# ekimb/rust-mdbg

Hardware: AMD Instinct MI355X
Metric: Gbases/s ingested to k-min-mer graph (higher is better)
Workload: dtype u64

## Files before the change

### include/mdbg_hip.h

```cpp
#ifndef MDBG_HIP_H
#define MDBG_HIP_H

#include <stddef.h>
#include <stdint.h>

#ifdef __cplusplus
extern "C" {
#endif

#define MDBG_ABI_VERSION 3

enum {
    MDBG_OK = 0,
    MDBG_E_PARAM = -1,
    MDBG_E_ALPHABET = -2,
    MDBG_E_CAPACITY = -3,
    MDBG_E_DEVICE = -4,
    MDBG_E_NOMEM = -5,
    MDBG_E_STATE = -6,
    MDBG_E_IO = -7
};

#define MDBG_MAX_L 255u
#define MDBG_MAX_MINABUND 65535u
// ... 183 lines not shown
    const uint64_t* step_offsets;
    const uint32_t* first_window; const uint32_t* step_windows; const uint32_t* unitig; const uint32_t* first_entry; const uint8_t* strand;
    const uint64_t* support_windows; const uint64_t* support_steps;
} mdbg_read_path_list;
int mdbg_graph_read_paths(mdbg_ctx* ctx, uint64_t first_read, uint64_t max_reads, mdbg_read_path_list* out);
int mdbg_graph_read_paths_device(mdbg_ctx* ctx, uint64_t first_read, uint64_t max_reads, mdbg_read_path_list* out);
int mdbg_read_paths_ms(mdbg_ctx* ctx, double* ms);

int mdbg_set_partition(mdbg_ctx* ctx, uint32_t world, uint32_t rank);
typedef struct mdbg_sketch_store {
    uint64_t n_minimizers, n_reads;
    const uint64_t* d_hashes;
    const uint32_t* d_positions;
    const uint64_t* d_read_offsets;
} mdbg_sketch_store;
int mdbg_sketch_view(mdbg_ctx* ctx, mdbg_sketch_store* out);
int mdbg_ingest_sketch(mdbg_ctx* ctx, const uint64_t* d_hashes, const uint32_t* d_positions, const uint64_t* d_read_offsets,
                       uint64_t n_reads, uint64_t first_read_ordinal);
int mdbg_store_reserve(mdbg_ctx* ctx, uint64_t n_minimizers_total, uint64_t n_reads_total);
int mdbg_sketch_reserve(mdbg_ctx* ctx, uint64_t n_minimizers, uint64_t** d_hashes, uint32_t** d_positions, uint64_t* region);
int mdbg_sketch_commit(mdbg_ctx* ctx, uint64_t region, uint64_t n_minimizers, const uint64_t* d_read_offsets, uint64_t n_reads,
                       uint64_t first_read_ordinal, uint64_t owned_windows);
int mdbg_owner_counts(mdbg_ctx* ctx, uint32_t world, uint64_t* counts);
int mdbg_owner_lists(mdbg_ctx* ctx, uint32_t world, uint64_t* counts, const uint32_t** d_lists);
int mdbg_sketch_commit_listed(mdbg_ctx* ctx, uint64_t region, uint64_t n_minimizers, const uint64_t* d_read_offsets, uint64_t n_reads,
                              uint64_t first_read_ordinal, const uint32_t* d_list, uint64_t n_list);
typedef struct mdbg_batch_info {
    uint64_t store_offset, n_minimizers, first_slot, n_reads, first_read_ordinal;
    const uint64_t* d_hashes;
    const uint32_t* d_positions;
    const uint64_t* d_read_offsets;
} mdbg_batch_info;
int mdbg_last_batch(mdbg_ctx* ctx, mdbg_batch_info* out);
int mdbg_finalize_begin(mdbg_ctx* ctx, uint64_t** d_bm_first, uint64_t** d_bm_solid, uint64_t* n_words);
int mdbg_finalize_end(mdbg_ctx* ctx, mdbg_nodes* out, const uint64_t** d_row, uint64_t* n_nodes_global);

int mdbg_sync(mdbg_ctx* ctx);
int mdbg_copy_to_host(mdbg_ctx* ctx, void* dst, const void* d_src, uint64_t nbytes);
int mdbg_copy_to_device(mdbg_ctx* ctx, void* d_dst, const void* src, uint64_t nbytes);

typedef struct mdbg_synth_params {
    uint64_t seed;
    uint64_t genome_len;
    uint64_t n_reads;
    uint32_t mean_len, sd_len, min_len, max_len;
    uint32_t err_ppm;
    uint32_t reserved;
} mdbg_synth_params;
int mdbg_synth_reads_device(mdbg_ctx* ctx, const mdbg_synth_params* sp, uint64_t first_read,
                            const uint8_t** d_bases, const uint64_t** d_offsets, uint64_t* n_bases);

int mdbg_dbg_segments_ms(mdbg_ctx* ctx, uint32_t world, uint32_t skip, const uint64_t* counts, const uint32_t* d_lists, double* out);

#ifdef __cplusplus
}
#endif
#endif
```

### rust_mdbg_amd/api.py

```python
import ctypes as C
import os

import numpy as np

_HERE = os.path.dirname(os.path.abspath(__file__))
_LIB = None

MDBG_OK, MDBG_E_PARAM, MDBG_E_ALPHABET, MDBG_E_CAPACITY, MDBG_E_DEVICE, MDBG_E_NOMEM, MDBG_E_STATE, MDBG_E_IO = 0, -1, -2, -3, -4, -5, -6, -7
FLAG_FORCE_GENERIC = 1
FLAG_KEEP_READS = 2


class MdbgError(RuntimeError):
    def __init__(self, code, msg):
        super().__init__("mdbg error %d: %s" % (code, msg))
        self.code = code


class Params(C.Structure):
    _fields_ = [("k", C.c_uint32), ("l", C.c_uint32), ("density", C.c_double), ("min_abundance", C.c_uint32),
                ("reads_already_hpc", C.c_uint32), ("device", C.c_int32), ("flags", C.c_uint32),
                ("table_capacity_hint", C.c_uint64), ("scheme", C.c_uint32), ("syncmer_s", C.c_uint32), ("reserved", C.c_uint64 * 3)]


# ... 89 lines not shown
                ("unitig", C.POINTER(C.c_uint64))]


class NodeSeqs(C.Structure):
    _fields_ = [("first_row", C.c_uint64), ("n_rows", C.c_uint64), ("n_bases", C.c_uint64), ("bases", C.POINTER(C.c_uint8)), ("offsets", C.POINTER(C.c_uint64))]


class SimplifyStep(C.Structure):
    _fields_ = [("kind", C.c_uint32), ("max_nodes", C.c_uint32), ("max_bases", C.c_uint64)]


class SimplifyStats(C.Structure):
    _fields_ = [("n_steps", C.c_uint32), ("n_compactions", C.c_uint32), ("unitigs_removed", C.POINTER(C.c_uint64)), ("nodes_removed", C.POINTER(C.c_uint64)),
                ("total_unitigs_removed", C.c_uint64), ("total_nodes_removed", C.c_uint64), ("n_rounds_total", C.c_uint32), ("n_syncs", C.c_uint32)]


MDBG_SIMPLIFY_TIPS, MDBG_SIMPLIFY_BUBBLES = 1, 2
MDBG_SIMPLIFY_COMPONENTS = 4
_T, _B = (MDBG_SIMPLIFY_TIPS, 10, 50000), (MDBG_SIMPLIFY_BUBBLES, 0, 100000)
MAGIC_SIMPLIFY_STEPS = [_T, _T, _B, _B, _T, _B, _B, _B, _T, _B, _T, (MDBG_SIMPLIFY_BUBBLES, 0, 1000000), (MDBG_SIMPLIFY_TIPS, 10, 150000),
                        (MDBG_SIMPLIFY_BUBBLES, 0, 1000000)]


def simplify_steps(steps):
    steps = [tuple(int(x) for x in s) for s in steps]
    if not steps:
        return None, 0
    return (SimplifyStep * len(steps))(*[SimplifyStep(k, mn, mb) for k, mn, mb in steps]), len(steps)


def unitig_name(i, circular):
    return "utg%07d%s" % (i + 1, "c" if circular else "l")


class PackedBatch(C.Structure):
    _fields_ = [("words", C.c_void_p), ("offsets", C.c_void_p), ("n_reads", C.c_uint64), ("exc_pos", C.c_void_p),
                ("exc_val", C.c_void_p), ("n_exc", C.c_uint64)]


class SynthParams(C.Structure):
    _fields_ = [("seed", C.c_uint64), ("genome_len", C.c_uint64), ("n_reads", C.c_uint64), ("mean_len", C.c_uint32),
                ("sd_len", C.c_uint32), ("min_len", C.c_uint32), ("max_len", C.c_uint32), ("err_ppm", C.c_uint32),
                ("reserved", C.c_uint32)]


EXPORTS = ["mdbg_abi_version", "mdbg_build_flags", "mdbg_create", "mdbg_destroy", "mdbg_finalize_device", "mdbg_finalize_gfa", "mdbg_nodes_digest", "mdbg_set_timing", "mdbg_ingest_batch", "mdbg_ingest_batch_device", "mdbg_sketch_only",
           "mdbg_finalize", "mdbg_reset", "mdbg_get_stats", "mdbg_strerror", "mdbg_last_error", "mdbg_sketch_device",
           "mdbg_insert_resident", "mdbg_route_pack", "mdbg_insert_records", "mdbg_sync", "mdbg_synth_reads_device", "mdbg_copy_to_host", "mdbg_copy_to_device",
           "mdbg_routed_export", "mdbg_resolve_first", "mdbg_resolve_meta", "mdbg_routed_keys", "mdbg_arena_reserve",
           "mdbg_set_partition", "mdbg_sketch_view", "mdbg_ingest_sketch", "mdbg_finalize_begin", "mdbg_finalize_end",
           "mdbg_store_reserve", "mdbg_sketch_reserve", "mdbg_sketch_commit", "mdbg_last_batch", "mdbg_owner_counts", "mdbg_graph_edges", "mdbg_graph_edges_device", "mdbg_graph_unitigs", "mdbg_graph_unitigs_device",
           "mdbg_graph_simplify", "mdbg_graph_simplify_device", "mdbg_graph_components", "mdbg_graph_components_device", "mdbg_graph_contigs", "mdbg_graph_contigs_device", "mdbg_kept_reads", "mdbg_contigs_ms", "mdbg_graph_node_seqs", "mdbg_graph_node_seqs_device", "mdbg_node_seqs_ms", "mdbg_graph_read_paths", "mdbg_graph_read_paths_device", "mdbg_read_paths_ms",
           "mdbg_ingest_batch_packed", "mdbg_ingest_batch_packed_device", "mdbg_sketch_packed_device", "mdbg_pack_device", "mdbg_query_batch", "mdbg_owner_lists", "mdbg_sketch_commit_listed", "mdbg_mark", "mdbg_rewind", "mdbg_set_lmer_filter",
           "mdbg_release_cached_memory", "mdbg_host_alloc", "mdbg_host_free", "mdbg_host_is_pinned", "mdbg_dbg_segments_ms"]


def lib_path():
    return os.path.join(_HERE, "libmdbg_hip.so")


def load_library():
    global _LIB
    if _LIB is not None:
        return _LIB
    p = lib_path()
    if not os.path.exists(p):
        raise ImportError("libmdbg_hip.so not built (%s); run `make -C rust_mdbg_amd/csrc`" % p)
    import sys
    if "torch" not in sys.modules and not os.environ.get("MDBG_NO_TORCH_PRELOAD"):
        import importlib.util
        if importlib.util.find_spec("torch") is not None:
            import torch
    L = C.CDLL(p)
    vp, u64, u32 = C.c_void_p, C.c_uint64, C.c_uint32
    L.mdbg_abi_version.restype = u32
    L.mdbg_build_flags.restype = u32
    L.mdbg_release_cached_memory.restype = u64
    L.mdbg_host_alloc.restype = vp
    L.mdbg_host_alloc.argtypes = [C.c_size_t]
    L.mdbg_host_free.restype = None
    L.mdbg_host_free.argtypes = [vp]
    L.mdbg_host_is_pinned.argtypes = [vp]
    L.mdbg_create.restype = vp
    L.mdbg_create.argtypes = [C.POINTER(Params), C.POINTER(C.c_int)]
    L.mdbg_destroy.restype = None
    L.mdbg_destroy.argtypes = [vp]
    L.mdbg_ingest_batch.argtypes = [vp, vp, vp, u64, u64]
    L.mdbg_ingest_batch_device.argtypes = [vp, vp, vp, u64, u64, u64]
    L.mdbg_sketch_device.argtypes = [vp, vp, vp, u64, u64, u64]
    L.mdbg_insert_resident.argtypes = [vp]
    L.mdbg_ingest_batch_packed.argtypes = [vp, C.POINTER(PackedBatch), u64]
    L.mdbg_ingest_batch_packed_device.argtypes = [vp, C.POINTER(PackedBatch), u64, u64]
    L.mdbg_sketch_packed_device.argtypes = [vp, C.POINTER(PackedBatch), u64, u64]
    L.mdbg_pack_device.argtypes = [vp, vp, u64, vp, vp, vp, u64, C.POINTER(u64)]
    L.mdbg_query_batch.argtypes = [vp, vp, vp, u64, C.POINTER(C.POINTER(u32)), C.POINTER(C.POINTER(u64)), C.POINTER(u64)]
    L.mdbg_query_batch.restype = C.c_int
    L.mdbg_sketch_only.argtypes = [vp, vp, vp, u64, C.POINTER(C.POINTER(u64)), C.POINTER(C.POINTER(u64)), C.POINTER(C.POINTER(u64)), C.POINTER(u64)]
    L.mdbg_finalize.argtypes = [vp, C.POINTER(Nodes)]
    L.mdbg_finalize_device.argtypes = [vp, C.POINTER(Nodes)]
    L.mdbg_finalize_gfa.argtypes = [vp, C.POINTER(Nodes)]
    L.mdbg_set_timing.argtypes = [vp, u32]
    L.mdbg_nodes_digest.argtypes = [vp, C.POINTER(Nodes), C.POINTER(C.c_uint64), C.POINTER(C.c_uint64)]
    L.mdbg_reset.argtypes = [vp, u32]
    L.mdbg_get_stats.argtypes = [vp, C.POINTER(Stats)]
    L.mdbg_strerror.restype = C.c_char_p
    L.mdbg_strerror.argtypes = [C.c_int]
    L.mdbg_last_error.restype = C.c_char_p
# ... 452 lines not shown
```

### rust_mdbg_amd/csrc/import_api.inc

```
int mdbg_set_partition(mdbg_ctx* c, uint32_t world, uint32_t rank) {
    if (!c) return MDBG_E_PARAM;
    MDBG_LOCK(c);
    if (world < 1 || world > 4096 || rank >= world) return fail(c, MDBG_E_PARAM, "bad partition");
    if (c->n_distinct || c->batches_inserted) return fail(c, MDBG_E_STATE, "set the partition before inserting");
    c->own_world = world; c->own_rank = rank;
    return MDBG_OK;
}

int mdbg_sketch_view(mdbg_ctx* c, mdbg_sketch_store* out) {
    if (!c || !out) return MDBG_E_PARAM;
    MDBG_LOCK(c);
    (void)hipSetDevice(c->dev);
    HIPCHK(c, hipStreamSynchronize(c->stream));
    out->n_minimizers = c->M; out->n_reads = c->n_slots;
    out->d_hashes = c->mh.as<u64>(); out->d_positions = c->mpos.as<u32>(); out->d_read_offsets = c->roff.as<u64>();
    return MDBG_OK;
}

int mdbg_ingest_sketch(mdbg_ctx* c, const uint64_t* d_hashes, const uint32_t* d_positions, const uint64_t* d_read_offsets, uint64_t n_reads,
                       uint64_t first_read_ordinal) {
    if (!c) return MDBG_E_PARAM;
    MDBG_LOCK(c);
    (void)hipSetDevice(c->dev);
    if (c->poisoned) return fail(c, MDBG_E_STATE, "context is in an error state");
// ... 159 lines not shown
}

static int batch_info_impl(mdbg_ctx* c, mdbg_batch_info* out, size_t which, bool sync = true) {
    if (!c || !out) return MDBG_E_PARAM;
    if (c->batches.empty() || (which != ~(size_t)0 && which >= c->batches.size())) return fail(c, MDBG_E_STATE, "no batch has been sketched or imported");
    MDBG_LOCK(c);
    (void)hipSetDevice(c->dev);
    if (sync) HIPCHK(c, hipStreamSynchronize(c->stream));
    const Batch& b = which == ~(size_t)0 ? c->batches.back() : c->batches[which];
    out->store_offset = b.m0; out->n_minimizers = b.m1 - b.m0; out->first_slot = b.slot0; out->n_reads = b.n_reads; out->first_read_ordinal = b.first_ordinal;
    out->d_hashes = c->mh.as<u64>() + b.m0; out->d_positions = c->mpos.as<u32>() + b.m0; out->d_read_offsets = c->roff.as<u64>() + b.slot0;
    return MDBG_OK;
}
int mdbg_last_batch(mdbg_ctx* c, mdbg_batch_info* out) { return batch_info_impl(c, out, ~(size_t)0); }

int mdbg_dbg_segments_ms(mdbg_ctx* c, uint32_t world, uint32_t skip, const uint64_t* counts, const uint32_t* d_lists, double* out) {
    if (!c || !counts || !d_lists || !out || world < 1 || world > OWNL_MAX_WORLD) return MDBG_E_PARAM;
    MDBG_LOCK(c);
    (void)hipSetDevice(c->dev);
    if (c->batches.empty()) return fail(c, MDBG_E_STATE, "no batch");
    const Batch& b = c->batches.back();
    hipStream_t s = c->stream;
    SegBuckets B{}; B.n = world; B.skip = skip;
    u64 total = 0;
    for (u32 r = 0; r < world; ++r) { B.start[r] = total; B.base[r] = b.m0; B.lim[r] = b.m1 - b.m0; total += counts[r]; }
    B.start[world] = total;
    out[0] = out[1] = 0; out[2] = (double)total; out[3] = 0;
    if (!total) return MDBG_OK;
    DevBuf tmp, misc, pay, scratch;
    HIPCHK(c, tmp.ensure((total / 1024 + 2) * 8, 0, s)); HIPCHK(c, misc.ensure((size_t)(OWNL_MAX_WORLD + 4) * 8, 0, s));
    HIPCHK(c, pay.ensure((b.m1 - b.m0) * 8 + 8, 0, s)); HIPCHK(c, scratch.ensure((b.m1 - b.m0) * 8 + 8, 0, s));
    hipEvent_t e0, e1; HIPCHK(c, hipEventCreate(&e0)); HIPCHK(c, hipEventCreate(&e1));
    u64 picks[OWNL_MAX_WORLD + 1] = {0};
    float best[2] = {1e30f, 1e30f};
    for (int rep = 0; rep < 3; ++rep)
        for (int side = 0; side < 2; ++side) {
            if (side) for (u32 r = 0; r < world; ++r) B.base[r] = 0;
            else for (u32 r = 0; r < world; ++r) B.base[r] = b.m0;
            HIPCHK(c, hipMemsetAsync(misc.p, 0, 8, s));
            HIPCHK(c, hipEventRecord(e0, s));
            launch_seg_prefix(d_lists, total, c->P.k, B, tmp.as<u64>(), misc.as<u64>(), misc.as<u64>() + 1, s);
            HIPCHK(c, hipMemcpyAsync(picks, misc.as<u64>() + 1, (size_t)(world + 1) * 8, hipMemcpyDeviceToHost, s));
            if (!side) HIPCHK(c, hipStreamSynchronize(s));
            launch_seg_copy(d_lists, total, c->P.k, B, tmp.as<u64>(), side ? scratch.as<u64>() : c->mh.as<u64>(), pay.as<u64>(), b.m1 - b.m0, side != 0, s);
            HIPCHK(c, hipEventRecord(e1, s));
            HIPCHK(c, hipStreamSynchronize(s));
            float ms = 0; HIPCHK(c, hipEventElapsedTime(&ms, e0, e1));
            if (ms < best[side]) best[side] = ms;
        }
    (void)hipEventDestroy(e0); (void)hipEventDestroy(e1);
    out[0] = best[0]; out[1] = best[1]; out[3] = (double)picks[world];
    return MDBG_OK;
}
```

### rust_mdbg_amd/csrc/owner.hip

```cpp
#include "mdbg_dev.h"
__global__ void owner_thresholds_kernel(double bound, u32 k, u32 world, u64* __restrict__ thr) {
    const u32 r = threadIdx.x + 1;
    if (threadIdx.x == 0) thr[0] = 0;
    thr += OWNER_THR_AT;
    if (r >= world) return;
    const double x = -expm1(log1p(-(double)r / (double)world) / (double)k);
    double v = x * bound;
    thr[r - 1] = v >= 18446744073709549568.0 ? ~0ull : (u64)v;
}
void launch_owner_thresholds(double bound, u32 k, u32 world, u64* thr, hipStream_t s) {
    if (world > 1) hipLaunchKernelGGL(owner_thresholds_kernel, dim3(1), dim3(64), 0, s, bound, k, world, thr);
}

__global__ __launch_bounds__(256) void count_owned_windows_kernel(const u64* __restrict__ mh, const u32* __restrict__ mread, const u64* __restrict__ roff, u64 i0, u64 i1,
                                                                  u32 k, u32 world, const u64* thr, u32 rank, u64* __restrict__ out) {
    constexpr int WPT = 4;
    const u64 b0 = i0 + (u64)blockIdx.x * (256 * WPT);
    u32 slot[WPT]; bool ok[WPT];
#pragma unroll
    for (int u = 0; u < WPT; ++u) { const u64 i = b0 + u * 256 + threadIdx.x; ok[u] = i < i1; slot[u] = ok[u] ? mread[i] : 0; }
    u32 mine = 0;
#pragma unroll
    for (int u = 0; u < WPT; ++u) {
        const u64 i = b0 + u * 256 + threadIdx.x;
// ... 223 lines not shown
        P0 += T;
    }
}
void launch_seg_copy(const u32* list, u64 n, u32 k, const SegBuckets& B, const u64* scan_tmp, u64* store, u64* payload, u64 payload_n, bool to_store, hipStream_t s) {
    if (n) hipLaunchKernelGGL(seg_copy_kernel, dim3((unsigned)((n + SEG_BLOCK - 1) / SEG_BLOCK)), dim3(256), 0, s, (const uint2*)list, n, k, B, scan_tmp, store, payload, payload_n, to_store ? 1u : 0u);
}

__device__ inline bool listed_check(u64 j) { return (((u32)j * 0x9E3779B1u) >> 28) == 0; }
struct ListedBatch { u64 start, m0, m1, first_ordinal; const u32* list; u32 slot0, n_reads; };
__global__ __launch_bounds__(256) void insert_listed_entries_kernel(TableArgs T, const u64* __restrict__ mh, u32* __restrict__ mread, const u64* __restrict__ roff,
                                                                    u64 m0, u64 m1, const u32* __restrict__ list, u64 n, u32 slot0, u32 n_reads, u64 first_ordinal,
                                                                    u32* __restrict__ cap_err, const ListedBatch* __restrict__ multi, u32 n_multi) {
    if (cap_err[1]) return;
    const u64 j = (u64)blockIdx.x * blockDim.x + threadIdx.x;
    const u32 k = T.ks.k;
    bool ok = j < n;
    u64 i = 0, rs = 0; u32 slot = 0;
    u64 jl = j;
    if (multi) {
        const u64 jw0 = (u64)blockIdx.x * blockDim.x + (threadIdx.x & ~63u);
        u64 jw = ((u64)__builtin_amdgcn_readfirstlane((u32)(jw0 >> 32)) << 32) | (u64)__builtin_amdgcn_readfirstlane((u32)jw0);
        if (jw >= n) jw = n - 1;
        u32 lo = 0, hi = n_multi - 1;
        while (lo < hi) { const u32 mid = (lo + hi + 1) >> 1; if (multi[mid].start <= jw) lo = mid; else hi = mid - 1; }
        if (ok && multi[lo + 1].start <= j) {
            hi = n_multi - 1;
            while (lo < hi) { const u32 mid = (lo + hi + 1) >> 1; if (multi[mid].start <= j) lo = mid; else hi = mid - 1; }
        }
        const ListedBatch b = multi[lo];
        m0 = b.m0; m1 = b.m1; list = b.list; slot0 = b.slot0; n_reads = b.n_reads; first_ordinal = b.first_ordinal; jl = j - b.start;
    }
    if (ok) {
        const uint2 e = ((const uint2*)list)[jl];
        i = m0 + e.x; slot = slot0 + e.y; ok = e.y < n_reads && i + k <= m1;
    }
    const u64* const w = mh + i;
    bool rev = false; u64 h = 0;
    if (ok) {
        const u64 w_first = w[0], w_last = w[k - 1];
        rs = roff[slot]; const u64 re = roff[slot + 1];
        ok = i >= rs && re - rs > k && i + k <= re;
        if (ok) {
            rev = w_first != w_last ? w_first > w_last : window_reversed(w, k);
            u64 smallest;
            h = key_hash_window_hbm(w, k, rev, smallest);
            ok = owner_of_min(smallest, k, OwnerSpec{T.own_world, T.own_thr}) == T.own_rank;
        }
    }
    wave_count_add(ok, T.own_inserted);
    const u64 win = i - rs;
    if (ok && win > WIN_MASK) { *cap_err = 1; ok = false; }
    const u64 ord = ((first_ordinal + (slot - slot0)) << WIN_BITS) | win;
    bool claimed, found;
    const u64 s = upsert_wave_h(T, ok, (u32)i, i, w, k, rev, h, claimed, found);
    if (claimed) { mread[i] = slot; if (T.claim) T.claim[i] = 1; }
    if (found) {
        atomicAdd(&T.tab[s].count, 1u);
        push_ordinal(T, s, ord);
    }
}
static void launch_listed_entries(const TableArgs& T, const u64* mh, u32* mread, const u64* roff, u64 m0, u64 m1, const u32* list, u64 n, u32 slot0, u32 n_reads, u64 first_ordinal,
                                  u32* cap_err, const ListedBatch* multi, u32 n_multi, hipStream_t s) {
    hipLaunchKernelGGL(insert_listed_entries_kernel, dim3((unsigned)((n + 255) / 256)), dim3(256), 0, s, T, mh, mread, roff, m0, m1, list, n, slot0, n_reads, first_ordinal, cap_err, multi, n_multi);
}
__global__ __launch_bounds__(256) void list_segments_kernel(const u32* __restrict__ list, u64 n, u32 n_spans, u32* __restrict__ seg) {
    const u64 j = (u64)blockIdx.x * blockDim.x + threadIdx.x;
    if (j >= n) return;
    const u32 last = n_spans - 1;
    u32 b = list[2 * j] / OWNL_SPAN; if (b > last) b = last;
    int pb = -1;
    if (j) { u32 q = list[2 * j - 2] / OWNL_SPAN; if (q > last) q = last; pb = (int)q; }
    for (int q = pb + 1; q <= (int)b; ++q) seg[q] = (u32)j;
}
u32 owner_list_spans(u64 n_minimizers) { return (u32)((n_minimizers + OWNL_SPAN - 1) / OWNL_SPAN); }
void launch_list_segments(const u32* list, u64 n, u32 n_spans, u32* seg, hipStream_t s) {
    (void)hipMemsetD32Async((hipDeviceptr_t)seg, (int)(u32)n, (size_t)n_spans + 1, s);
    if (n && n_spans) hipLaunchKernelGGL(list_segments_kernel, dim3((unsigned)((n + 255) / 256)), dim3(256), 0, s, list, n, n_spans, seg);
}
static size_t listed_span_lds(const TableArgs& T) { return ((size_t)OWNL_SPAN + T.ks.k) * sizeof(u64) + OWNL_SPAN; }
__global__ __launch_bounds__(256) void insert_listed_span_kernel(TableArgs T, const u64* __restrict__ mh, u32* __restrict__ mread, const u64* __restrict__ roff,
                                                                 u64 m0, u64 m1, const u32* __restrict__ list, const u32* __restrict__ seg, u64 n, u32 slot0,
                                                                 u32 n_reads, u64 first_ordinal, u32* __restrict__ cap_err) {
    extern __shared__ u64 sh_keys[];
    if (cap_err[1]) return;
    const u32 q = blockIdx.x, k = T.ks.k;
    const u32 s0 = seg[q], s1 = seg[q + 1];
    const u64 b0 = m0 + (u64)q * OWNL_SPAN;
    u8* const cl = (u8*)(sh_keys + OWNL_SPAN + k);
    const u64 span_n = m1 - b0 < (u64)OWNL_SPAN ? m1 - b0 : (u64)OWNL_SPAN;
    if (s0 >= s1 || s1 > n) {
        if (T.claim) for (u32 li = threadIdx.x; li < span_n; li += 256) T.claim[b0 + li] = 0;
        return;
    }
    const u64 lim = b0 + OWNL_SPAN + k - 1 < m1 ? b0 + OWNL_SPAN + k - 1 : m1;
    for (u64 t = b0 + threadIdx.x; t < lim; t += 256) sh_keys[t - b0] = mh[t];
    if (T.claim) for (int u = threadIdx.x; u < OWNL_SPAN / 8; u += 256) ((u64*)cl)[u] = 0;
    __syncthreads();
    for (u32 base = s0; base < s1; base += 256) {
        const u32 j = base + threadIdx.x;
        bool ok = j < s1;
        u32 li = 0; u64 i = 0;
        u32 slot = 0; u64 rs = 0;
        if (ok) {
            const uint2 e = ((const uint2*)list)[j];
            li = e.x; ok = li / OWNL_SPAN == q && e.y < n_reads; li -= q * OWNL_SPAN; i = b0 + li; slot = slot0 + e.y;
        }
        if (ok) {
            rs = roff[slot]; const u64 re = roff[slot + 1];
            ok = i >= rs && re - rs > k && i + k <= re && (!listed_check(j) || window_owner(sh_keys + li, k, OwnerSpec{T.own_world, T.own_thr}) == T.own_rank);
        }
        wave_count_add(ok, T.own_inserted);
        const u64 win = i - rs;
        if (ok && win > WIN_MASK) { *cap_err = 1; ok = false; }
        const u64 ord = ((first_ordinal + (slot - slot0)) << WIN_BITS) | win;
        bool claimed, found;
        const u64 s = upsert_wave(T, ok, li, i, sh_keys + li, k, claimed, found);
        if (claimed) { mread[i] = slot; if (T.claim) cl[li] = 1; }
        if (found) {
            atomicAdd(&T.tab[s].count, 1u);
            push_ordinal(T, s, ord);
        }
    }
    if (T.claim) {
        __syncthreads();
        for (u32 li = threadIdx.x; li < span_n; li += 256) T.claim[b0 + li] = cl[li];
    }
}
constexpr u64 LISTED_SPAN_MIN = 150;
bool listed_per_entry(const TableArgs& T, u64 m0, u64 m1, u64 n, bool have_seg) {
    return !have_seg || listed_span_lds(T) > 64 * 1024 || n < (u64)owner_list_spans(m1 - m0) * LISTED_SPAN_MIN;
}
void launch_insert_listed(const TableArgs& T, const u64* mh, u32* mread, const u64* roff, u64 m0, u64 m1, const u32* list, const u32* seg, u64 n, u32 slot0,
                          u32 n_reads, u64 first_ordinal, u32* cap_err, hipStream_t s) {
    if (!n) return;
    if (!listed_per_entry(T, m0, m1, n, seg != nullptr))
        hipLaunchKernelGGL(insert_listed_span_kernel, dim3(owner_list_spans(m1 - m0)), dim3(256), listed_span_lds(T), s, T, mh, mread, roff, m0, m1, list, seg, n, slot0, n_reads, first_ordinal, cap_err);
    else
        launch_listed_entries(T, mh, mread, roff, m0, m1, list, n, slot0, n_reads, first_ordinal, cap_err, nullptr, 0u, s);
}
void launch_insert_listed_multi(const TableArgs& T, const u64* mh, u32* mread, const u64* roff, const ListedBatch* d_batches, u32 n_batches, u64 total, u32* cap_err, hipStream_t s) {
    if (!total) return;
    launch_listed_entries(T, mh, mread, roff, 0ull, 0ull, nullptr, total, 0u, 0u, 0ull, cap_err, d_batches, n_batches, s);
}
```

### rust_mdbg_amd/csrc/table.hip

```cpp
#include "mdbg_dev.h"

struct __attribute__((aligned(32))) Slot {
    u64 word;
    u64 m1;
    u64 m2;
    u32 count;
    u32 pad;
};
constexpr u64 EMPTY = ~0ull;
constexpr u64 HMUL = 0x9E3779B97F4A7C15ull;

struct KeySrc {
    const u64* mh;
    const u64* arena;
    u32 k;
};

__device__ inline u64 load_relaxed(const u64* p) { return __hip_atomic_load(p, __ATOMIC_RELAXED, __HIP_MEMORY_SCOPE_AGENT); }

__device__ inline u64 rep_elem(const KeySrc& ks, u64 word, u32 j) {
    const u32 rep = (u32)word;
    if (word & (1ull << 33)) return ks.arena[(u64)rep * (ks.k + 2) + j];
    return (word & (1ull << 32)) ? ks.mh[(u64)rep + ks.k - 1 - j] : ks.mh[(u64)rep + j];
}
// ... 148 lines not shown
}

constexpr u32 OWNER_BINS = 65536, OWNER_THR_AT = 1, OWNER_TAB_AT = 64, OWNER_PARAM_WORDS = OWNER_TAB_AT + OWNER_BINS / 8;
struct OwnerSpec { u32 world; const u64* thr; };
__device__ inline u32 owner_of_min(u64 m, u32 k, OwnerSpec os);
__device__ inline u32 window_owner(const u64* __restrict__ w, u32 k, OwnerSpec os) {
    if (os.world <= 1) return 0;
    u64 m = w[0];
    for (u32 j = 1; j < k; ++j) { const u64 x = w[j]; m = x < m ? x : m; }
    return owner_of_min(m, k, os);
}
__device__ inline u32 owner_of_min(u64 m, u32 k, OwnerSpec os) {
    (void)k;
    if (os.world <= 1) return 0;
    if (!os.thr) return (u32)__umul64hi(fmix64(m), (u64)os.world);
    const u64 mul = os.thr[0];
    if (mul) {
        const u64 bin = __umul64hi(m, mul);
        const u32 o = ((const u8*)(os.thr + OWNER_TAB_AT))[bin < OWNER_BINS ? bin : OWNER_BINS - 1];
        return o < os.world ? o : os.world - 1;
    }
    const u64* const thr = os.thr + OWNER_THR_AT;
    u32 lo = 0, hi = os.world - 1;
    while (lo < hi) { const u32 mid = (lo + hi) >> 1; if (thr[mid] <= m) lo = mid + 1; else hi = mid; }
    return lo;
}

struct OwnerCodes { u64 mul; const u64* thr; u32 world; };
__device__ inline OwnerCodes owner_codes_of(OwnerSpec os) { OwnerCodes c; c.thr = os.thr; c.world = os.world; c.mul = os.thr ? os.thr[0] : 0; return c; }
__device__ inline u16 owner_code(u64 v, const OwnerCodes& c) {
    if (c.mul) { const u64 bin = __umul64hi(v, c.mul); return (u16)(bin < OWNER_BINS ? bin : OWNER_BINS - 1); }
    const u64* const thr = c.thr + OWNER_THR_AT;
    u32 lo = 0, hi = c.world - 1;
    while (lo < hi) { const u32 mid = (lo + hi) >> 1; if (thr[mid] <= v) lo = mid + 1; else hi = mid; }
    return (u16)lo;
}
__device__ inline u32 owner_of_code(u16 code, const OwnerCodes& c) {
    if (!c.mul) return code;
    const u32 o = ((const u8*)(c.thr + OWNER_TAB_AT))[code];
    return o < c.world ? o : c.world - 1;
}
template <class ValueFn, class ValidFn>
__device__ inline const u16* span_min_codes(ValueFn value, ValidFn valid, u32 nv, u32 k, const OwnerCodes& c, u16* a, u16* b, u32& p) {
    for (u32 t = threadIdx.x; t < nv; t += 256) a[t] = valid(t) ? owner_code(value(t), c) : (u16)0xFFFFu;
    __syncthreads();
    for (p = 1; 2 * p <= k; p *= 2) {
        for (u32 t = threadIdx.x; t < nv; t += 256) { const u16 x = a[t], y = t + p < nv ? a[t + p] : (u16)0xFFFFu; b[t] = x < y ? x : y; }
        __syncthreads();
        u16* const sw = a; a = b; b = sw;
    }
    return a;
}

__device__ inline u64 upsert_wave_h(const TableArgs& T, bool act, u32 li, u64 i, const u64* w, u32 k, bool rev, u64 h, bool& claimed, bool& found);
__device__ inline u64 upsert_wave(const TableArgs& T, bool act, u32 li, u64 i, const u64* w, u32 k, bool& claimed, bool& found) {
    bool rev = false; u64 h = 0;
    if (act) { rev = window_reversed(w, k); h = key_hash_window(w, k, rev); }
    return upsert_wave_h(T, act, li, i, w, k, rev, h, claimed, found);
}
__device__ inline u64 upsert_wave_h(const TableArgs& T, bool act, u32 li, u64 i, const u64* w, u32 k, bool rev, u64 h, bool& claimed, bool& found) {
    const int lane = threadIdx.x & 63;
    const u64 fp = (h >> 34) & T.fp_mask;
    const u64 myword_lo = ((u64)rev << 32) | (u64)(u32)i;
    auto eq = [&](u64 word) { return same_key_window(T.ks, word, w, rev); };
    u64 s = act ? home_slot(h, T.cap) : 0, word = EMPTY, probes = 0;
    claimed = false;
    bool cand = false;
    if (act) {
        for (; probes <= T.cap; ++probes) {
            u64 wv = load_relaxed(&T.tab[s].word);
            if (wv == EMPTY) {
                const u64 old = atomicCAS((unsigned long long*)&T.tab[s].word, (unsigned long long)EMPTY, (unsigned long long)((fp << 34) | myword_lo));
                if (old == EMPTY) { wave_agg_inc(T.n_distinct); claimed = true; break; }
                wv = old;
            }
            if ((wv >> 34) == fp) { word = wv; cand = true; break; }
            s = s + 1 == T.cap ? 0 : s + 1;
        }
        if (!claimed && !cand) { *T.probe_err = 1; s = ~0ull; }
    }
    const bool cross = rev != ((word & (1ull << 32)) != 0);
    const u32 rep = (u32)word;
    const u32 p_li = (u32)__shfl_up((int)li, 1, 64), p_rep = (u32)__shfl_up((int)rep, 1, 64);
    const int p_info = __shfl_up((int)((cand && !(word & (1ull << 33)) ? 1 : 0) | (cross ? 2 : 0)), 1, 64);
    const bool link = cand && !T.no_chain && lane > 0 && !(word & (1ull << 33)) && (p_info & 1) && p_li + 1 == li && ((p_info >> 1) & 1) == (int)cross &&
                      rep == (cross ? p_rep - 1u : p_rep + 1u);
    bool pass = false;
    if (cand) pass = link ? T.ks.mh[(u64)rep + (cross ? 0u : k - 1u)] == w[k - 1] : eq(word);
    const u64 heads = __ballot(!link), fails = __ballot(cand && !pass);
    found = pass;
    if (link && pass) {
        const int hp = 63 - __clzll((unsigned long long)(heads & ((2ull << lane) - 1ull)));
        found = ((fails >> hp) & ((2ull << (lane - hp)) - 1ull)) == 0;
    }
    if (T.link_ctr) { const u64 lm = __ballot(link && found); if (lane == 0 && lm) atomicAdd(T.link_ctr, (unsigned long long)__popcll(lm)); }
    if (cand && !found) {
        const bool skip = !link;
        s = upsert_slot_from(T, h, myword_lo, eq, claimed, skip ? (s + 1 == T.cap ? 0 : s + 1) : s, probes + (skip ? 1 : 0));
        found = !claimed && s != ~0ull;
    }
    return s;
}

constexpr int OWN_SPAN = 2048;
static size_t insert_windows_lds(const TableArgs& T) {
    const size_t codes = T.own_world > 1 && T.own_thr ? 2 * ((size_t)OWN_SPAN + T.ks.k) * sizeof(u16) : 0;
    return (OWN_SPAN + T.ks.k) * sizeof(u64) + OWN_SPAN * sizeof(u16) + 16 + OWN_SPAN + codes;
}
__global__ __launch_bounds__(256) void insert_windows_kernel(TableArgs T, const u64* __restrict__ mh, const u32* __restrict__ mread,
                                                                   const u64* __restrict__ roff, u64 i0, u64 i1, u32 slot0, u64 first_ordinal,
                                                                   u32* __restrict__ cap_err, const u64* __restrict__ i1_dev, u64 n_lim) {
    extern __shared__ u64 sh_keys[];
    if (cap_err[1]) return;
    if (i1_dev) { i1 = *i1_dev; if (i0 + (u64)blockIdx.x * OWN_SPAN >= i1) return; }
    const u32 k = T.ks.k;
    u16* const list = (u16*)(sh_keys + OWN_SPAN + k);
    u32* const n_own = (u32*)(list + OWN_SPAN);
    u8* const cl = (u8*)(n_own + 4);
    const u64 b0 = i0 + (u64)blockIdx.x * OWN_SPAN;
    const u64 lim = b0 + OWN_SPAN + k - 1 < i1 ? b0 + OWN_SPAN + k - 1 : i1;
    for (u64 t = b0 + threadIdx.x; t < lim; t += 256) sh_keys[t - b0] = mh[t];
    if (threadIdx.x == 0) *n_own = 0;
    if (T.claim) for (int u = threadIdx.x; u < OWN_SPAN / 8; u += 256) ((u64*)cl)[u] = 0;
    __syncthreads();
    const bool by_codes = T.own_world > 1 && T.own_thr != nullptr;
    const u16* mc = nullptr; u32 pc = 1; OwnerCodes oc{};
    if (by_codes) {
        u16* const ca = (u16*)(cl + OWN_SPAN);
        oc = owner_codes_of(OwnerSpec{T.own_world, T.own_thr});
        const u32 n_st = (u32)(lim - b0);
        mc = span_min_codes([&](u32 t) { return sh_keys[t]; }, [&](u32 t) { return t < n_st; }, OWN_SPAN + k - 1, k, oc, ca, ca + (OWN_SPAN + k), pc);
    }
#pragma unroll
    for (int u = 0; u < OWN_SPAN / 256; ++u) {
        const u32 li = u * 256 + threadIdx.x;
        const u64 i = b0 + li;
        bool mine = false;
        bool own = i + k <= i1;
        if (own && T.own_world > 1) {
            if (by_codes) { const u16 x = mc[li], y = mc[li + k - pc]; own = owner_of_code(x < y ? x : y, oc) == T.own_rank; }
            else own = window_owner(sh_keys + li, k, OwnerSpec{T.own_world, T.own_thr}) == T.own_rank;
        }
        if (own) {
            const u32 slot = mread[i];
            const u64 rs = roff[slot], re = roff[slot + 1];
            mine = re - rs > k && i + k <= re;
        }
        const u64 m = __ballot(mine);
        u32 base = 0;
        if ((threadIdx.x & 63) == 0 && m) base = atomicAdd(n_own, (u32)__popcll(m));
        base = __shfl(base, 0, 64);
        if (mine) list[base + __popcll(m & ((1ull << (threadIdx.x & 63)) - 1))] = (u16)li;
    }
    __syncthreads();
    const u32 n = *n_own;
    if (threadIdx.x == 0 && n && T.own_world > 1) atomicAdd((unsigned long long*)ctr_shard(T.own_inserted), (unsigned long long)n);
    for (u32 j0 = 0; j0 < n; j0 += 256) {
        const u32 j = j0 + threadIdx.x;
        bool act = j < n;
        const u32 li = act ? list[j] : 0u;
        const u64 i = b0 + li;
        u64 ord = 0;
        if (act) {
            const u32 slot = mread[i];
            const u64 win = i - roff[slot];
            if (win > WIN_MASK) { *cap_err = 1; act = false; }
            ord = ((first_ordinal + (slot - slot0)) << WIN_BITS) | win;
        }
        bool claimed, found;
        const u64 s = upsert_wave(T, act, li, i, sh_keys + li, k, claimed, found);
        if (claimed && T.claim) cl[li] = 1;
        if (found) {
            atomicAdd(&T.tab[s].count, 1u);
            push_ordinal(T, s, ord);
        }
    }
    if (T.claim) {
        __syncthreads();
        const u64 hi = i1 - b0 < (u64)OWN_SPAN ? i1 - b0 : (u64)OWN_SPAN;
        for (u32 li = threadIdx.x; li < hi && li < n_lim - (u64)blockIdx.x * OWN_SPAN; li += 256) T.claim[b0 + li] = cl[li];
    }
}
void launch_insert_windows(const TableArgs& T, const u64* mh, const u32* mread, const u64* roff, u64 i0, u64 i1, u32 slot0,
                           u64 first_ordinal, u64* n_windows, u32* cap_err, hipStream_t s, const u64* i1_dev = nullptr, u64 n_starts = 0) {
    if (i1 <= i0) return;
    (void)n_windows;
    const u64 n = n_starts ? n_starts : i1 - i0;
    hipLaunchKernelGGL(insert_windows_kernel, dim3((unsigned)((n + OWN_SPAN - 1) / OWN_SPAN)), dim3(256), insert_windows_lds(T), s, T, mh, mread, roff, i0, i1, slot0, first_ordinal, cap_err, i1_dev, n);
}

__global__ __launch_bounds__(256) void insert_records_kernel(TableArgs T, u64 r0, u64 r1, u64* __restrict__ n_windows) {
    const u64 r = r0 + (u64)blockIdx.x * blockDim.x + threadIdx.x;
    if (r >= r1) return;
    const u32 k = T.ks.k;
    const u64* key = T.ks.arena + r * (k + 2);
    const u64 h = key[k + 1];
    bool claimed;
    const u64 s = upsert_slot(T, h, (1ull << 33) | (u64)(u32)r, [&](u64 word) { return same_key_window(T.ks, word, key, false); }, claimed);
    if (claimed || s == ~0ull) return;
    atomicAdd(&T.tab[s].count, 1u);
    push_ordinal(T, s, key[k]);
    (void)n_windows;
}
void launch_insert_records(const TableArgs& T, u64 r0, u64 r1, u64* n_windows, hipStream_t s) {
    if (r1 <= r0) return;
    hipLaunchKernelGGL(insert_records_kernel, dim3((unsigned)((r1 - r0 + 255) / 256)), dim3(256), 0, s, T, r0, r1, n_windows);
}

__global__ void clear_table_kernel(Slot* __restrict__ tab, u64 cap, u64* __restrict__ mx, u64 n_mx, ZeroList z) {
    const u64 stride = (u64)gridDim.x * blockDim.x;
    {
        const u64 i0 = (u64)blockIdx.x * blockDim.x + threadIdx.x;
#pragma unroll
        for (int r = 0; r < 6; ++r) for (u64 i = i0; i < z.n[r]; i += stride) z.p[r][i] = 0;
        if (i0 == 0 && z.set_p) *z.set_p = z.set_v;
    }
    for (u64 i = (u64)blockIdx.x * blockDim.x + threadIdx.x; i < cap; i += stride) {
        uint4* p = (uint4*)(tab + i);
        p[0] = make_uint4(0xFFFFFFFFu, 0xFFFFFFFFu, 0xFFFFFFFFu, 0xFFFFFFFFu);
        p[1] = make_uint4(0xFFFFFFFFu, 0xFFFFFFFFu, 0u, 0u);
    }
    for (u64 i = (u64)blockIdx.x * blockDim.x + threadIdx.x; i < n_mx; i += stride) mx[i] = EMPTY;
}
// ... 177 lines not shown
```

Baseline: 2511.

## Confirm hash-table key matches cooperatively across the wavefront instead of per lane

Replaces the per-thread full-key comparison in the upsert path with a wave-cooperative confirm routine. Candidate lanes are compacted with ballot/permute, and groups of L lanes compare each key in two-word chunks, so one lane no longer walks a k-long key serially. The collision probe loop is restructured into a wave-wide while loop that calls the cooperative confirm at each step. A standalone confirm-keys kernel and API entry are added for testing. The cost is extra permute and ballot traffic plus wave-uniform looping, which may hurt when few lanes need confirmation or k is small.

New measurement: 2570 (median of 6 runs). 2.4% higher.

```diff
diff --git a/include/mdbg_hip.h b/include/mdbg_hip.h
--- a/include/mdbg_hip.h
+++ b/include/mdbg_hip.h
@@ -259,6 +259,8 @@
 
 int mdbg_dbg_segments_ms(mdbg_ctx* ctx, uint32_t world, uint32_t skip, const uint64_t* counts, const uint32_t* d_lists, double* out);
 
+int mdbg_dbg_confirm_keys(mdbg_ctx* ctx, const uint64_t* d_hashes, uint32_t k, const uint32_t* d_pairs, uint64_t n, uint8_t* d_verdicts);
+
 #ifdef __cplusplus
 }
 #endif
diff --git a/rust_mdbg_amd/api.py b/rust_mdbg_amd/api.py
--- a/rust_mdbg_amd/api.py
+++ b/rust_mdbg_amd/api.py
@@ -165,7 +165,7 @@
            "mdbg_store_reserve", "mdbg_sketch_reserve", "mdbg_sketch_commit", "mdbg_last_batch", "mdbg_owner_counts", "mdbg_graph_edges", "mdbg_graph_edges_device", "mdbg_graph_unitigs", "mdbg_graph_unitigs_device",
            "mdbg_graph_simplify", "mdbg_graph_simplify_device", "mdbg_graph_components", "mdbg_graph_components_device", "mdbg_graph_contigs", "mdbg_graph_contigs_device", "mdbg_kept_reads", "mdbg_contigs_ms", "mdbg_graph_node_seqs", "mdbg_graph_node_seqs_device", "mdbg_node_seqs_ms", "mdbg_graph_read_paths", "mdbg_graph_read_paths_device", "mdbg_read_paths_ms",
            "mdbg_ingest_batch_packed", "mdbg_ingest_batch_packed_device", "mdbg_sketch_packed_device", "mdbg_pack_device", "mdbg_query_batch", "mdbg_owner_lists", "mdbg_sketch_commit_listed", "mdbg_mark", "mdbg_rewind", "mdbg_set_lmer_filter",
-           "mdbg_release_cached_memory", "mdbg_host_alloc", "mdbg_host_free", "mdbg_host_is_pinned", "mdbg_dbg_segments_ms"]
+           "mdbg_release_cached_memory", "mdbg_host_alloc", "mdbg_host_free", "mdbg_host_is_pinned", "mdbg_dbg_segments_ms", "mdbg_dbg_confirm_keys"]
 
 
 def lib_path():
diff --git a/rust_mdbg_amd/csrc/import_api.inc b/rust_mdbg_amd/csrc/import_api.inc
--- a/rust_mdbg_amd/csrc/import_api.inc
+++ b/rust_mdbg_amd/csrc/import_api.inc
@@ -235,3 +235,13 @@
     out[0] = best[0]; out[1] = best[1]; out[3] = (double)picks[world];
     return MDBG_OK;
 }
+
+int mdbg_dbg_confirm_keys(mdbg_ctx* c, const uint64_t* d_hashes, uint32_t k, const uint32_t* d_pairs, uint64_t n, uint8_t* d_verdicts) {
+    if (!c || !d_hashes || !d_pairs || !d_verdicts || k < 2 || k > 4096) return MDBG_E_PARAM;
+    MDBG_LOCK(c);
+    (void)hipSetDevice(c->dev);
+    launch_confirm_keys(d_hashes, k, d_pairs, n, d_verdicts, c->stream);
+    HIPCHK(c, hipGetLastError());
+    HIPCHK(c, hipStreamSynchronize(c->stream));
+    return MDBG_OK;
+}
diff --git a/rust_mdbg_amd/csrc/owner.hip b/rust_mdbg_amd/csrc/owner.hip
--- a/rust_mdbg_amd/csrc/owner.hip
+++ b/rust_mdbg_amd/csrc/owner.hip
@@ -299,7 +299,7 @@
     if (ok && win > WIN_MASK) { *cap_err = 1; ok = false; }
     const u64 ord = ((first_ordinal + (slot - slot0)) << WIN_BITS) | win;
     bool claimed, found;
-    const u64 s = upsert_wave_h(T, ok, (u32)i, i, w, k, rev, h, claimed, found);
+    const u64 s = upsert_wave_h(T, ok, (u32)i, i, mh, k, rev, h, claimed, found);
     if (claimed) { mread[i] = slot; if (T.claim) T.claim[i] = 1; }
     if (found) {
         atomicAdd(&T.tab[s].count, 1u);
@@ -361,7 +361,7 @@
         if (ok && win > WIN_MASK) { *cap_err = 1; ok = false; }
         const u64 ord = ((first_ordinal + (slot - slot0)) << WIN_BITS) | win;
         bool claimed, found;
-        const u64 s = upsert_wave(T, ok, li, i, sh_keys + li, k, claimed, found);
+        const u64 s = upsert_wave(T, ok, li, i, sh_keys, k, claimed, found);
         if (claimed) { mread[i] = slot; if (T.claim) cl[li] = 1; }
         if (found) {
             atomicAdd(&T.tab[s].count, 1u);
diff --git a/rust_mdbg_amd/csrc/table.hip b/rust_mdbg_amd/csrc/table.hip
--- a/rust_mdbg_amd/csrc/table.hip
+++ b/rust_mdbg_amd/csrc/table.hip
@@ -224,33 +224,85 @@
     return a;
 }
 
-__device__ inline u64 upsert_wave_h(const TableArgs& T, bool act, u32 li, u64 i, const u64* w, u32 k, bool rev, u64 h, bool& claimed, bool& found);
-__device__ inline u64 upsert_wave(const TableArgs& T, bool act, u32 li, u64 i, const u64* w, u32 k, bool& claimed, bool& found) {
+constexpr int CONFIRM_G = 2;
+__device__ inline bool confirm_keys_wave(const KeySrc& ks, bool need, u64 word, const u64* wb, u32 li, bool rev) {
+    const u64 todo = __ballot(need);
+    if (!todo) return false;
+    const u32 k = ks.k;
+    const u32 lane = threadIdx.x & 63;
+    const u32 n = (u32)__popcll((unsigned long long)todo);
+    const u32 L = k >= 127 ? 64u : (k + 1) / 2, P = 64u / L, n_slots = (n + P - 1) / P;
+    const u32 sub = lane / L, t = lane - sub * L;
+    const u64 below = (1ull << lane) - 1ull;
+    const u32 num = need ? (u32)__popcll((unsigned long long)(todo & below)) : n + (u32)__popcll((unsigned long long)(~todo & below));
+    const bool in_arena = (word & (1ull << 33)) != 0;
+    const bool cross = in_arena ? rev : rev != ((word & (1ull << 32)) != 0);
+    const int c_rep = __builtin_amdgcn_ds_permute((int)(num * 4u), (int)(u32)word);
+    const int c_li = __builtin_amdgcn_ds_permute((int)(num * 4u), (int)li);
+    const int c_info = __builtin_amdgcn_ds_permute((int)(num * 4u), (cross ? 1 : 0) | (in_arena ? 2 : 0));
+    bool equal = false;
+    for (u32 s0 = 0; s0 < n_slots; s0 += CONFIRM_G) {
+        u64 differ[CONFIRM_G];
+#pragma unroll
+        for (int g = 0; g < CONFIRM_G; ++g) differ[g] = 0;
+        for (u32 j0 = 0; j0 < k; j0 += 2 * L) {
+            const u32 e = j0 + 2 * t + 2 <= k ? j0 + 2 * t : k - 2;
+            u64x2_a8 a[CONFIRM_G];
+#pragma unroll
+            for (int g = 0; g < CONFIRM_G; ++g) {
+                const u32 q = (s0 + g) * P + sub;
+                const int from = (int)((sub < P && q < n ? q : 0u) * 4u);
+                const u32 r = (u32)__builtin_amdgcn_ds_bpermute(from, c_rep);
+                const u64* const rp = (__builtin_amdgcn_ds_bpermute(from, c_info) & 2) ? ks.arena + (u64)r * (k + 2) : ks.mh + r;
+                a[g] = *(const u64x2_a8*)(rp + e);
+            }
+#pragma unroll
+            for (int g = 0; g < CONFIRM_G; ++g) {
+                const u32 q = (s0 + g) * P + sub;
+                const bool vote = sub < P && q < n;
+                const int from = (int)((vote ? q : 0u) * 4u);
+                const u64* const own = wb + (u32)__builtin_amdgcn_ds_bpermute(from, c_li);
+                const bool crs = (__builtin_amdgcn_ds_bpermute(from, c_info) & 1) != 0;
+                const u64 o0 = crs ? own[k - 1 - e] : own[e], o1 = crs ? own[k - 2 - e] : own[e + 1];
+                differ[g] |= __ballot(vote && ((a[g].x ^ o0) | (a[g].y ^ o1)) != 0);
+                }
+        }
+#pragma unroll
+        for (int g = 0; g < CONFIRM_G; ++g) {
+            const u32 at = num - (s0 + g) * P;
+            equal = need && at < P ? ((differ[g] >> (at * L)) << (64u - L)) == 0 : equal;
+        }
+    }
+    return equal;
+}
+
+__device__ inline u64 upsert_wave_h(const TableArgs& T, bool act, u32 li, u64 i, const u64* wb, u32 k, bool rev, u64 h, bool& claimed, bool& found);
+__device__ inline u64 upsert_wave(const TableArgs& T, bool act, u32 li, u64 i, const u64* wb, u32 k, bool& claimed, bool& found) {
     bool rev = false; u64 h = 0;
-    if (act) { rev = window_reversed(w, k); h = key_hash_window(w, k, rev); }
-    return upsert_wave_h(T, act, li, i, w, k, rev, h, claimed, found);
-}
-__device__ inline u64 upsert_wave_h(const TableArgs& T, bool act, u32 li, u64 i, const u64* w, u32 k, bool rev, u64 h, bool& claimed, bool& found) {
+    if (act) { rev = window_reversed(wb + li, k); h = key_hash_window(wb + li, k, rev); }
+    return upsert_wave_h(T, act, li, i, wb, k, rev, h, claimed, found);
+}
+__device__ inline u64 upsert_wave_h(const TableArgs& T, bool act, u32 li, u64 i, const u64* wb, u32 k, bool rev, u64 h, bool& claimed, bool& found) {
     const int lane = threadIdx.x & 63;
-    const u64 fp = (h >> 34) & T.fp_mask;
-    const u64 myword_lo = ((u64)rev << 32) | (u64)(u32)i;
-    auto eq = [&](u64 word) { return same_key_window(T.ks, word, w, rev); };
+    const u32 fp = (u32)((h >> 34) & T.fp_mask);
     u64 s = act ? home_slot(h, T.cap) : 0, word = EMPTY, probes = 0;
     claimed = false;
     bool cand = false;
-    if (act) {
+    auto probe = [&]() {
+        cand = false;
         for (; probes <= T.cap; ++probes) {
             u64 wv = load_relaxed(&T.tab[s].word);
             if (wv == EMPTY) {
-                const u64 old = atomicCAS((unsigned long long*)&T.tab[s].word, (unsigned long long)EMPTY, (unsigned long long)((fp << 34) | myword_lo));
+                const u64 old = atomicCAS((unsigned long long*)&T.tab[s].word, (unsigned long long)EMPTY, (unsigned long long)(((u64)fp << 34) | ((u64)rev << 32) | (u64)(u32)i));
                 if (old == EMPTY) { wave_agg_inc(T.n_distinct); claimed = true; break; }
                 wv = old;
             }
-            if ((wv >> 34) == fp) { word = wv; cand = true; break; }
+            if ((u32)(wv >> 34) == fp) { word = wv; cand = true; break; }
             s = s + 1 == T.cap ? 0 : s + 1;
         }
         if (!claimed && !cand) { *T.probe_err = 1; s = ~0ull; }
-    }
+    };
+    if (act) probe();
     const bool cross = rev != ((word & (1ull << 32)) != 0);
     const u32 rep = (u32)word;
     const u32 p_li = (u32)__shfl_up((int)li, 1, 64), p_rep = (u32)__shfl_up((int)rep, 1, 64);
@@ -258,7 +310,9 @@
     const bool link = cand && !T.no_chain && lane > 0 && !(word & (1ull << 33)) && (p_info & 1) && p_li + 1 == li && ((p_info >> 1) & 1) == (int)cross &&
                       rep == (cross ? p_rep - 1u : p_rep + 1u);
     bool pass = false;
-    if (cand) pass = link ? T.ks.mh[(u64)rep + (cross ? 0u : k - 1u)] == w[k - 1] : eq(word);
+    if (link) pass = T.ks.mh[(u64)rep + (cross ? 0u : k - 1u)] == wb[(u64)li + k - 1];
+    const bool head_eq = confirm_keys_wave(T.ks, cand && !link, word, wb, li, rev);
+    if (cand && !link) pass = head_eq;
     const u64 heads = __ballot(!link), fails = __ballot(cand && !pass);
     found = pass;
     if (link && pass) {
@@ -266,12 +320,31 @@
         found = ((fails >> hp) & ((2ull << (lane - hp)) - 1ull)) == 0;
     }
     if (T.link_ctr) { const u64 lm = __ballot(link && found); if (lane == 0 && lm) atomicAdd(T.link_ctr, (unsigned long long)__popcll(lm)); }
-    if (cand && !found) {
-        const bool skip = !link;
-        s = upsert_slot_from(T, h, myword_lo, eq, claimed, skip ? (s + 1 == T.cap ? 0 : s + 1) : s, probes + (skip ? 1 : 0));
-        found = !claimed && s != ~0ull;
+    bool walk = cand && !found, need = walk && link;
+    if (walk && !need) { s = s + 1 == T.cap ? 0 : s + 1; ++probes; }
+    while (__ballot(walk)) {
+        if (walk && !need) { probe(); need = walk = cand; }
+        const bool eq = confirm_keys_wave(T.ks, need, word, wb, li, rev);
+        if (need) {
+            if (eq) { found = true; walk = false; }
+            else { s = s + 1 == T.cap ? 0 : s + 1; ++probes; }
+        }
+        need = false;
     }
     return s;
+}
+__global__ __launch_bounds__(256) void confirm_keys_kernel(const u64* __restrict__ mh, u32 k, const u32* __restrict__ pairs, u64 n, u8* __restrict__ out) {
+    const u64 j = (u64)blockIdx.x * blockDim.x + threadIdx.x;
+    const bool ok = j < n;
+    u32 rep = 0, rrev = 0, own = 0, orev = 0, active = 0;
+    if (ok) { rep = pairs[5 * j]; rrev = pairs[5 * j + 1]; own = pairs[5 * j + 2]; orev = pairs[5 * j + 3]; active = pairs[5 * j + 4]; }
+    KeySrc ks; ks.mh = mh; ks.arena = mh; ks.k = k;
+    const bool eq = confirm_keys_wave(ks, ok && active != 0, ((u64)(rrev != 0) << 32) | rep, mh, own, orev != 0);
+    if (ok) out[j] = eq ? 1 : 0;
+}
+void launch_confirm_keys(const u64* mh, u32 k, const u32* pairs, u64 n, u8* out, hipStream_t s) {
+    if (!n) return;
+    hipLaunchKernelGGL(confirm_keys_kernel, dim3((unsigned)((n + 255) / 256)), dim3(256), 0, s, mh, k, pairs, n, out);
 }
 
 constexpr int OWN_SPAN = 2048;
@@ -340,7 +413,7 @@
             ord = ((first_ordinal + (slot - slot0)) << WIN_BITS) | win;
         }
         bool claimed, found;
-        const u64 s = upsert_wave(T, act, li, i, sh_keys + li, k, claimed, found);
+        const u64 s = upsert_wave(T, act, li, i, sh_keys, k, claimed, found);
         if (claimed && T.claim) cl[li] = 1;
         if (found) {
             atomicAdd(&T.tab[s].count, 1u);
```
